# Ryan-Yanlong/DREAM-GNN

Hardware: AMD Instinct MI355X
Metric: GCMC+FGCN SpMM edges/sec and achieved HBM GB/s at 1/2/4/8 MI355X (higher is better)
Workload: dtype f32

## Files before the change

dream_gnn_amd/csrc/dgmi_api.hip:

```cpp
#include <hip/hip_runtime.h>
#include <limits.h>
#include <stdlib.h>
#include <string.h>

#include "dgmi.h"
#include "dgmi_bf16.h"
#include "dgmi_keep.h"
#include "dgmi_layout.h"
#include "dgmi_scale.h"
#include "dgmi_kernels.h"
#include "dgmi_tuning.h"

namespace {

inline hipStream_t as_stream(dgmi_stream_t s) { return static_cast<hipStream_t>(s); }

inline int from_hip(hipError_t e) { return e == hipSuccess ? DGMI_OK : DGMI_ERR_LAUNCH; }

long long env_ll(const char* name, long long dflt) {
  const char* e = getenv(name);
  return e != nullptr && e[0] != '\0' ? atoll(e) : dflt;
}

}

namespace dgmi {

Tuning& tuning() {
  static Tuning t = [] {
    Tuning v;
    v.sliced_rows = (int)env_ll("DGMI_SLICED_ROWS", 0);
    v.sliced_touch_lead = (int)env_ll("DGMI_SLICED_PF", -1);
    v.sliced_lpr = (int)env_ll("DGMI_SLICED_LPR", 0);
    v.sliced_no_off32 = getenv("DGMI_NO_OFF32") != nullptr ? 1 : 0;
    v.sliced_chunk_rows = env_ll("DGMI_SLICED_CHUNK_ROWS", 0);
    v.sliced_taper_rows = env_ll("DGMI_SLICED_TAPER_ROWS", 0);
    v.sliced_owned = (int)env_ll("DGMI_SLICED_OWNED", -1);
    v.sliced_owned_grid = (int)env_ll("DGMI_SLICED_OWNED_GRID", 0);
    v.sliced_owned_wgs = (int)env_ll("DGMI_SLICED_OWNED_WGS", 0);
    v.sliced_owned_rows = (int)env_ll("DGMI_SLICED_OWNED_ROWS", 0);
    v.sliced_owned_lds_rows = env_ll("DGMI_SLICED_OWNED_LDS_ROWS", 0);
    v.sliced_owned_workers = (int)env_ll("DGMI_SLICED_OWNED_WORKERS", 0);
    v.sliced_owned_slices = (int)env_ll("DGMI_SLICED_OWNED_SLICES", 0);
    v.sliced_owned_scaled = (int)env_ll("DGMI_SLICED_OWNED_SCALED", -1);
    v.sliced_owned_lag = (int)env_ll("DGMI_SLICED_OWNED_LAG", -2);
    v.sliced_owned_spin_ticks = env_ll("DGMI_SLICED_OWNED_SPIN_TICKS", 0);
    v.select_window_min = env_ll("DGMI_SELECT_WINDOW_MIN", 0);
    v.select_narrow_window = env_ll("DGMI_SELECT_NARROW_WINDOW", 0) != 0 ? 1 : 0;
    v.sort_plain_tiles = env_ll("DGMI_SORT_PLAIN_TILES", 0) != 0 ? 1 : 0;
    v.knn_screen_first = env_ll("DGMI_KNN_SCREEN_V1", 0) != 0 ? 1 : 0;
    v.knn_pool_chunks = env_ll("DGMI_KNN_POOL_CHUNKS", 0);
    return v;
  }();
  return t;
}

}

extern "C" {

DGMI_API int dgmi_set_tuning(const char* name, int64_t value) {
  if (name == nullptr) return DGMI_ERR_INVALID_ARG;
  dgmi::Tuning& t = dgmi::tuning();
  if (strcmp(name, "sliced_rows") == 0) t.sliced_rows = (int)value;
  else if (strcmp(name, "sliced_touch_lead") == 0) t.sliced_touch_lead = (int)value;
  else if (strcmp(name, "sliced_lpr") == 0) t.sliced_lpr = (int)value;
  else if (strcmp(name, "sliced_no_off32") == 0) t.sliced_no_off32 = value != 0;
  else if (strcmp(name, "sliced_chunk_rows") == 0) t.sliced_chunk_rows = value;
  else if (strcmp(name, "sliced_taper_rows") == 0) t.sliced_taper_rows = value;
  else if (strcmp(name, "sliced_owned") == 0) t.sliced_owned = (int)value;
  else if (strcmp(name, "sliced_owned_grid") == 0) t.sliced_owned_grid = (int)value;
  else if (strcmp(name, "sliced_owned_wgs") == 0) t.sliced_owned_wgs = (int)value;
  else if (strcmp(name, "sliced_owned_rows") == 0) t.sliced_owned_rows = (int)value;
  else if (strcmp(name, "sliced_owned_lds_rows") == 0) t.sliced_owned_lds_rows = value;
  else if (strcmp(name, "sliced_owned_workers") == 0) t.sliced_owned_workers = (int)value;
  else if (strcmp(name, "sliced_owned_slices") == 0) t.sliced_owned_slices = (int)value;
  else if (strcmp(name, "sliced_owned_scaled") == 0) t.sliced_owned_scaled = (int)value;
  else if (strcmp(name, "sliced_owned_lag") == 0) t.sliced_owned_lag = (int)value;
  else if (strcmp(name, "sliced_owned_spin_ticks") == 0) t.sliced_owned_spin_ticks = value;
  else if (strcmp(name, "select_window_min") == 0) t.select_window_min = value;
  else if (strcmp(name, "select_narrow_window") == 0) t.select_narrow_window = value != 0;
  else if (strcmp(name, "sort_plain_tiles") == 0) t.sort_plain_tiles = value != 0;
  else if (strcmp(name, "knn_screen_first") == 0) t.knn_screen_first = value != 0;
  else if (strcmp(name, "knn_pool_chunks") == 0) t.knn_pool_chunks = value;
  else return DGMI_ERR_INVALID_ARG;
  return DGMI_OK;
}

DGMI_API int dgmi_abi_version(void) { return DGMI_ABI_VERSION; }

DGMI_API const char* dgmi_status_string(int status) {
  switch (status) {
    case DGMI_OK: return "ok";
    case DGMI_ERR_INVALID_ARG: return "invalid argument (null pointer, negative size or ld < F)";
    case DGMI_ERR_TOO_LARGE: return "size does not fit the int32 id space";
    case DGMI_ERR_WORKSPACE: return "workspace missing or too small";
    case DGMI_ERR_LAUNCH: return "HIP launch failed";
    case DGMI_ERR_NO_DEVICE: return "no gfx950 device visible";
    default: return "unknown dgmi status";
  }
}

DGMI_API int dgmi_device_ok(void) {
  int n = 0;
  if (hipGetDeviceCount(&n) != hipSuccess || n <= 0) return 0;
  int dev = 0;
  if (hipGetDevice(&dev) != hipSuccess) return 0;
  hipDeviceProp_t prop;
  if (hipGetDeviceProperties(&prop, dev) != hipSuccess) return 0;
  return strncmp(prop.gcnArchName, "gfx950", 6) == 0 ? 1 : 0;
}

DGMI_API int dgmi_csr_from_coo_i32(const int32_t* row, const int32_t* col, int64_t E, int64_t n_rows,
                          int64_t n_cols, int32_t* indptr, int32_t* indices, int32_t* eid, void* workspace,
                          size_t* workspace_bytes, dgmi_stream_t stream) {
  if (E < 0 || n_rows < 0 || workspace_bytes == nullptr) return DGMI_ERR_INVALID_ARG;
  if (E > INT32_MAX || n_rows >= INT32_MAX || n_cols >= INT32_MAX) return DGMI_ERR_TOO_LARGE;
  if (workspace != nullptr) {
    if (indptr == nullptr) return DGMI_ERR_INVALID_ARG;
    if (E > 0 && (row == nullptr || col == nullptr || indices == nullptr || eid == nullptr))
      return DGMI_ERR_INVALID_ARG;
  }
  size_t need = 0;
  hipError_t err = dgmi::csr_from_coo_i32(row, col, E, n_rows, n_cols, indptr, indices, eid, nullptr,
                                          &need, as_stream(stream));
  if (err != hipSuccess) return DGMI_ERR_LAUNCH;
  if (workspace == nullptr) {
    *workspace_bytes = need;
    return DGMI_OK;
  }
// ... 487 lines not shown
```

dream_gnn_amd/csrc/dgmi_owned.hip:

```cpp
#include <hip/hip_runtime.h>
#include <limits.h>
#include <stdint.h>

#include <map>
#include <mutex>
#include <type_traits>
#include <utility>

#include "dgmi_owned_common.h"
#include "dgmi_owned_kernel.h"
#include "dgmi_sliced_common.h"

namespace dgmi {
namespace {

constexpr int64_t kOwnedSpinTicks = 3000;
constexpr int64_t kOwnedMinRows = 32768;
constexpr int kOwnedLag = -1;
constexpr int kOwnedWideSlices = 16;
constexpr int kOwnedAssumedCus = 256;

template <int LPR, int VALS, bool OFF32, int WAVES>
__global__ __launch_bounds__(kWave* WAVES, WAVES == kOwnedWaves ? 4 : 6) void spmm_owned_kernel(
    const int32_t* __restrict__ segptr, const int32_t* __restrict__ indices, const float* __restrict__ X, int64_t ldx,
    const float* __restrict__ dst_scale, float* __restrict__ Y, int64_t ldy, int64_t n_dst, int F, OwnedPlan pl,
    unsigned* __restrict__ arrive, int lag, int64_t spin_ticks, int workers, Epilogue ep) {
  owned_body<OwnedRowF32, LPR, VALS, OFF32, WAVES, true>(segptr, indices, X, ldx, dst_scale, Y, ldy, n_dst, F, pl, arrive, lag,
                                                         spin_ticks, workers, ep);
}

template <int LPR, int VALS, bool OFF32>
__global__ __launch_bounds__(kWave* kOwnedWaves, 4) void spmm_owned_bf16_kernel(
    const int32_t* __restrict__ segptr, const int32_t* __restrict__ indices, const uint16_t* __restrict__ X, int64_t ldx,
    const float* __restrict__ dst_scale, float* __restrict__ Y, int64_t ldy, int64_t n_dst, int F, OwnedPlan pl,
    unsigned* __restrict__ arrive, int lag, int64_t spin_ticks, int workers, Epilogue ep) {
  owned_body<OwnedRowBf16, LPR, VALS, OFF32, kOwnedWaves, false>(segptr, indices, X, ldx, dst_scale, Y, ldy, n_dst, F, pl, arrive,
                                                                 lag, spin_ticks, workers, ep);
}

constexpr size_t kOwnedScaleLdsBytes = sizeof(float) << kScaleBits;
template <int LPR, int VALS>
__global__ __launch_bounds__(kWave* kOwnedWaves, 4) void spmm_owned_scaled_kernel(
    const int32_t* __restrict__ segptr, const int32_t* __restrict__ indices, const float* __restrict__ X, int64_t ldx,
    const float* __restrict__ dst_scale, float* __restrict__ Y, int64_t ldy, int64_t n_dst, int F, OwnedPlan pl, int workers,
    Epilogue ep, const float* __restrict__ table, int n_codes) {
  owned_body<OwnedRowF32, LPR, VALS, true, kOwnedWaves, false, true>(segptr, indices, X, ldx, dst_scale, Y, ldy, n_dst, F, pl, nullptr,
                                                                     -1, 0, workers, ep, table, n_codes);
}

constexpr bool owned_scaled_built(int lpr) { return lpr == 16 || lpr == 32; }

template <int LPR>
hipError_t launch_owned_scaled(const SlicedArgs& a, const OwnedPlan& pl, int64_t grid, hipStream_t s) {
  const int workers = tuning().sliced_owned_workers > 0 && tuning().sliced_owned_workers < kOwnedWorkers ? tuning().sliced_owned_workers : 0;
  const size_t lds = pl.lds_bytes + kOwnedScaleLdsBytes;
#define DGMI_OWNED_SCALED(V)                                                                                              \
  do {                                                                                                                    \
    auto kern = &spmm_owned_scaled_kernel<LPR, V>;                                                                        \
    static const hipError_t attr =                                                                                        \
        hipFuncSetAttribute(reinterpret_cast<const void*>(kern), hipFuncAttributeMaxDynamicSharedMemorySize, 160 << 10);  \
    if (attr != hipSuccess) return attr;                                                                                  \
    hipLaunchKernelGGL(kern, dim3((unsigned)grid), dim3(kWave* kOwnedWaves), lds, s, a.segptr, a.indices,                 \
                       static_cast<const float*>(a.X), a.ldx, a.dst_scale, a.Y, a.ldy, a.n_dst, (int)a.F, pl, workers, a.ep, \
                       a.scale_table, a.n_codes);                                                                         \
  } while (0)
  if (a.id_mult) DGMI_OWNED_SCALED(2); else DGMI_OWNED_SCALED(0);
#undef DGMI_OWNED_SCALED
  return hipGetLastError();
}

template <typename Row, int LPR, int VALS, bool OFF32, int WAVES>
constexpr auto owned_kernel() {
  if constexpr (std::is_same<Row, OwnedRowBf16>::value)
    return &spmm_owned_bf16_kernel<LPR, VALS, OFF32>;
  else
    return &spmm_owned_kernel<LPR, VALS, OFF32, WAVES>;
}

int device_cus() {
  static const int cus = [] {
    int dev = 0, n = 0;
    if (hipGetDevice(&dev) != hipSuccess || hipDeviceGetAttribute(&n, hipDeviceAttributeMultiprocessorCount, dev) != hipSuccess)
      return 0;
    return n;
  }();
  return cus;
}

int owned_class_form(const OwnedPlan& pl, bool id_mult, int64_t table_bytes, int x_bytes) {
  const auto mib = [&](int64_t lo, int64_t hi) { return table_bytes >= (lo << 20) && table_bytes <= (hi << 20); };
  if (x_bytes == 2) {
    if (pl.slices != kOwnedSlices || pl.col_rounds != 1) return 0;
    if (pl.row_rounds == 1 && !id_mult && mib(16, 32)) return 1;
    if (pl.row_rounds == 2 && !id_mult && mib(8, 16)) return 1;
    if (pl.row_rounds == 2 && id_mult && mib(16, 32)) return 1;
    if (pl.row_rounds == 1 && id_mult && mib(8, 16)) return 1;
    return 0;
  }
  if (x_bytes != 4) return 0;
  if (pl.slices == kOwnedSlices) {
    if (pl.col_rounds == 1 && pl.row_rounds == 2 && !id_mult && mib(16, 32)) return 1;
    if (pl.col_rounds == 2 && pl.row_rounds == 1 && id_mult && mib(48, 64)) return 1;
    if (pl.col_rounds == 1 && pl.row_rounds == 1 && id_mult && mib(16, 32)) return 1;
  }
  if (pl.slices == kOwnedWideSlices && pl.col_rounds == 1 && pl.row_rounds == 1 && !id_mult && mib(48, 64)) return 1;
  return 0;
}

int owned_class_phase_tasks(const OwnedPlan& pl, bool id_mult, int64_t table_bytes, int x_bytes) {
  if (x_bytes != 4) return kOwnedPhaseTasks;
  const auto mib = [&](int64_t lo, int64_t hi) { return table_bytes >= (lo << 20) && table_bytes <= (hi << 20); };
  if (pl.slices != kOwnedSlices) return kOwnedPhaseTasks;
  if (pl.col_rounds == 2 && pl.row_rounds == 1 && id_mult && mib(48, 64)) return kOwnedPhaseTasksMult;
  if (pl.col_rounds == 1 && pl.row_rounds == 1 && id_mult && mib(16, 32)) return kOwnedPhaseTasksMult;
  return kOwnedPhaseTasks;
}

bool owned_coresident(const void* kern, int threads, size_t lds, int wgs) {
  static std::mutex mu;
  static std::map<std::pair<const void*, size_t>, int> known;
  std::lock_guard<std::mutex> lock(mu);
// ... 25 lines not shown
    auto kern = owned_kernel<Row, LPR, V, O, WAVES>();                                                                    \
    static const hipError_t attr = hipFuncSetAttribute(reinterpret_cast<const void*>(kern),                               \
                                                       hipFuncAttributeMaxDynamicSharedMemorySize, (160 << 10) / kWgsPerCu); \
    if (attr != hipSuccess) return attr;                                                                                  \
    if (kWgsPerCu > 1 && !owned_coresident(reinterpret_cast<const void*>(kern), kWave * WAVES, pl.lds_bytes, kWgsPerCu)) { \
      *resident = false;                                                                                                  \
      return hipSuccess;                                                                                                  \
    }                                                                                                                     \
    if (lag >= 0) {                                                            \
      const hipError_t err = hipMemsetAsync(arrive, 0, sizeof(unsigned) * 8 * (size_t)pl.phases, s);                      \
      if (err != hipSuccess) return err;                                                                                  \
    }                                                                                                                     \
    hipLaunchKernelGGL(kern, dim3((unsigned)grid), dim3(kWave* WAVES), pl.lds_bytes, s, a.segptr, a.indices,              \
                       static_cast<const typename Row::Elem*>(a.X), a.ldx, a.dst_scale, a.Y, a.ldy, a.n_dst, (int)a.F, pl, \
                       arrive, lag, spin_ticks, workers, a.ep);                                                           \
    }                                                                                                                     \
  } while (0)
  if (a.id_mult) {
    if (off32) DGMI_OWNED(2, true); else DGMI_OWNED(2, false);
  } else {
    if (off32) DGMI_OWNED(0, true); else DGMI_OWNED(0, false);
  }
#undef DGMI_OWNED
  return hipGetLastError();
}

template <typename Row, int WAVES>
hipError_t launch_owned_width(const SlicedArgs& a, const OwnedPlan& pl, int lpr, int64_t grid, bool off32, int lag,
                              int64_t spin_ticks, hipStream_t s, bool* resident) {
  switch (lpr) {
    case 8: return launch_owned<Row, 8, WAVES>(a, pl, grid, off32, lag, spin_ticks, s, resident);
    case 16: return launch_owned<Row, 16, WAVES>(a, pl, grid, off32, lag, spin_ticks, s, resident);
    case 32: return launch_owned<Row, 32, WAVES>(a, pl, grid, off32, lag, spin_ticks, s, resident);
    case 64:
      if constexpr (Row::kMaxLpr >= 64)
        return launch_owned<Row, 64, WAVES>(a, pl, grid, off32, lag, spin_ticks, s, resident);
      else
        return hipErrorInvalidValue;
    default: return hipErrorInvalidValue;
  }
}

bool owned_class_scaled(const OwnedPlan& pl, bool id_mult, int64_t table_bytes) {
  const auto mib = [&](int64_t lo, int64_t hi) { return table_bytes >= (lo << 20) && table_bytes <= (hi << 20); };
  if (pl.slices == kOwnedSlices) {
    if (pl.col_rounds == 1 && pl.row_rounds == 2 && !id_mult && mib(16, 32)) return true;
    if (pl.col_rounds == 2 && pl.row_rounds == 1 && id_mult && mib(48, 64)) return true;
    if (pl.col_rounds == 1 && pl.row_rounds == 1 && id_mult && mib(16, 32)) return true;
  }
  if (pl.slices == kOwnedWideSlices && pl.col_rounds == 1 && pl.row_rounds == 1 && !id_mult && mib(48, 64)) return true;
  return false;
}

hipError_t owned_try(const SlicedArgs& a, hipStream_t s, bool* taken, bool launch);

}

hipError_t spmm_owned_try(const SlicedArgs& a, hipStream_t s, bool* taken) {
  *taken = false;
  if (a.scale_table != nullptr) return hipErrorInvalidValue;
  return owned_try(a, s, taken, true);
}

bool spmm_owned_scaled_takes(const SlicedArgs& a) {
  bool taken = false;
  return a.scale_table != nullptr && owned_try(a, nullptr, &taken, false) == hipSuccess && taken;
}

hipError_t spmm_owned_scaled(const SlicedArgs& a, hipStream_t s, bool* taken) {
  *taken = false;
  if (a.scale_table == nullptr) return hipErrorInvalidValue;
  return owned_try(a, s, taken, true);
}

namespace {

hipError_t owned_try(const SlicedArgs& a, hipStream_t s, bool* taken, bool launch) {
  *taken = false;
  const Tuning& tune = tuning();
  if (tune.sliced_owned == 0) return hipSuccess;
  if ((a.x_bytes != 4 && a.x_bytes != 2) || a.vals != nullptr || a.src_scale != nullptr || a.n_keep != 0 || a.n_slices < 1 || a.n_slices > kOwnedMaxSlices ||
      tune.sliced_chunk_rows > 0 || a.chunk_rows < a.n_dst || a.n_dst == 0 || a.F == 0)
    return hipSuccess;
  if (a.x_bytes == 2 && tune.sliced_owned_slices > 0) return hipSuccess;
  const int64_t grid = tune.sliced_owned_grid > 0 ? tune.sliced_owned_grid : device_cus();
  if (grid < 1) return hipSuccess;
  const int lpr = sliced_lpr(a.F, a.n_src, a.n_slices, a.n_dst, a.full_width, a.n_keep, a.x_bytes, tune.sliced_lpr);
  const int slices = (int)a.n_slices;
  const int cols = 16 / a.x_bytes;
  const int64_t table_bytes = a.n_src * a.ldx * (int64_t)a.x_bytes;
  OwnedPlan pl = owned_plan(a.n_dst, a.F, lpr, grid, tune.sliced_owned_rows, tune.sliced_owned_lds_rows, 1, kOwnedPhaseTasks, slices, cols);
  const int phase_tasks = a.n_dst < kOwnedMinRows ? kOwnedPhaseTasks : owned_class_phase_tasks(pl, a.id_mult, table_bytes, a.x_bytes);
  if (pl.ok && phase_tasks != kOwnedPhaseTasks)
    pl = owned_plan(a.n_dst, a.F, lpr, grid, tune.sliced_owned_rows, tune.sliced_owned_lds_rows, 1, phase_tasks, slices, cols);
  if (!pl.ok || pl.lds_bytes > (size_t)(160 << 10)) return hipSuccess;
  const int rule = a.n_dst < kOwnedMinRows ? 0 : owned_class_form(pl, a.id_mult, table_bytes, a.x_bytes);
  if (tune.sliced_owned != 1 && rule == 0) return hipSuccess;
  const bool off32 = !tune.sliced_no_off32 && (a.n_src * a.ldx + a.F) * a.x_bytes < ((int64_t)1 << 32);
  bool resident = true;
  if (a.scale_table != nullptr) {
    const bool wanted = tune.sliced_owned_scaled == 1 ||
                        (tune.sliced_owned_scaled < 0 && (tune.sliced_owned == 1 || (rule == 1 && owned_class_scaled(pl, a.id_mult, table_bytes))));
    if (!wanted || a.x_bytes != 4 || a.n_src > ((int64_t)1 << kScaleShift) || a.n_codes < 1 || a.n_codes > (1 << kScaleBits) ||
        !off32 || !owned_scaled_built(lpr) || pl.lds_bytes + kOwnedScaleLdsBytes > (size_t)(160 << 10) || tune.sliced_owned_lag >= 0 ||
        tune.sliced_owned_wgs == 2)
      return hipSuccess;
    *taken = true;
    if (!launch) return hipSuccess;
    return lpr == 16 ? launch_owned_scaled<16>(a, pl, grid, s) : launch_owned_scaled<32>(a, pl, grid, s);
  }
  if (!launch) return hipSuccess;
  if (a.x_bytes == 2) {
    *taken = true;
    return launch_owned_width<OwnedRowBf16, kOwnedWaves>(a, pl, lpr, grid, off32, -1, 0, s, &resident);
  }
  const auto arrive_fits = [&](const OwnedPlan& p) {
    return sizeof(unsigned) * 8 * (size_t)p.phases <= sizeof(float) * (size_t)a.n_slices * (size_t)a.n_dst * (size_t)a.ldp;
  };
  if (!arrive_fits(pl)) return hipSuccess;
  const int form = tune.sliced_owned_wgs == 1 || tune.sliced_owned_wgs == 2 ? tune.sliced_owned_wgs : (rule == 2 ? 2 : 1);
  const int64_t spin = tune.sliced_owned_spin_ticks > 0 ? tune.sliced_owned_spin_ticks : kOwnedSpinTicks;
  const int lag = tune.sliced_owned_lag >= -1 ? tune.sliced_owned_lag : kOwnedLag;
  *taken = true;
  if (form == 2) {
    const int64_t grid2 = tune.sliced_owned_grid > 0 ? grid : 2 * grid;
    const OwnedPlan pl2 = owned_plan(a.n_dst, a.F, lpr, grid2, tune.sliced_owned_rows, tune.sliced_owned_lds_rows, 2, kOwnedPhaseTasks, slices);
    if (pl2.ok && pl2.lds_bytes <= (size_t)(80 << 10) && arrive_fits(pl2)) {
      const hipError_t err = launch_owned_width<OwnedRowF32, kOwnedPairWaves>(a, pl2, lpr, grid2, off32, lag, spin, s, &resident);
      if (err != hipSuccess || resident) return err;
    }
  }
  return launch_owned_width<OwnedRowF32, kOwnedWaves>(a, pl, lpr, grid, off32, lag, spin, s, &resident);
}

}

int sliced_layout_slices(int64_t n_dst, int64_t n_src, int64_t F, bool id_mult) {
  const Tuning& tune = tuning();
  if (n_dst < 1 || n_src < 1 || F < 1 || F % 4 != 0 || tune.sliced_owned == 0 || tune.sliced_chunk_rows > 0) return kOwnedSlices;
  const int forced = tune.sliced_owned_slices;
  const int slices = forced > 0 ? (forced < kOwnedMaxSlices ? forced : kOwnedMaxSlices) : kOwnedWideSlices;
  if (slices == kOwnedSlices) return kOwnedSlices;
  if (n_dst * slices >= INT32_MAX || n_dst * slices * F * (int64_t)sizeof(float) > ((int64_t)4096 << 20)) return kOwnedSlices;
  const int64_t grid = tune.sliced_owned_grid > 0 ? tune.sliced_owned_grid : (device_cus() > 0 ? device_cus() : kOwnedAssumedCus);
  const int lpr = sliced_lpr(F, n_src, slices, n_dst, false, 0, 4, tune.sliced_lpr);
  const OwnedPlan pl = owned_plan(n_dst, F, lpr, grid, tune.sliced_owned_rows, tune.sliced_owned_lds_rows, 1, kOwnedPhaseTasks, slices);
  if (!pl.ok || pl.lds_bytes > (size_t)(160 << 10)) return kOwnedSlices;
  if (forced > 0) return slices;
  if (n_dst < kOwnedMinRows) return kOwnedSlices;
  return owned_class_form(pl, id_mult, n_src * F * (int64_t)sizeof(float), 4) == 1 ? slices : kOwnedSlices;
}

}
```

dream_gnn_amd/csrc/dgmi_owned_common.h:

```cpp
#pragma once
#include <hip/hip_runtime.h>
#include <stddef.h>
#include <stdint.h>

namespace dgmi {

constexpr int kOwnedSlices = 8;
constexpr int kOwnedMaxSlices = 64;
constexpr int kOwnedWaves = 16;
constexpr int kOwnedWorkers = kOwnedWaves - 1;
constexpr int kOwnedPairWaves = 12;
constexpr int64_t kOwnedLdsRowBytes = 144 << 10;
constexpr int kOwnedMaxPhases = 128;
constexpr int kOwnedPhaseTasks = 24;
constexpr int kOwnedPhaseTasksMult = 32;
constexpr int kOwnedMaxRows = 8;

struct OwnedPlan {
  bool ok;
  int lpr, G, R;
  int col_rounds, row_rounds, phases;
  int slices;
  int64_t wg_rows;
  int64_t active;
  int round_rows;
  int tasks;
  int64_t n_dst;
  size_t lds_bytes;
};

struct OwnedPhase {
  int col_round, row_round, slice;
};

struct OwnedTask {
  int64_t row0;
  int lds_row;
  int rows;
};

__host__ __device__ constexpr int owned_form_waves(int wgs_per_cu) { return wgs_per_cu == 2 ? kOwnedPairWaves : kOwnedWaves; }

__host__ __device__ inline OwnedPlan owned_plan(int64_t n_dst, int64_t F, int lpr, int64_t grid, int R_req, int64_t lds_rows_cap,
                                                int wgs_per_cu = 1, int phase_tasks_target = kOwnedPhaseTasks,
                                                int slices = kOwnedSlices, int cols_per_lane = 4) {
  OwnedPlan p{};
  p.ok = false;
  p.n_dst = n_dst;
  if (n_dst < 1 || F < 1 || grid < 1 || (wgs_per_cu != 1 && wgs_per_cu != 2) || (lpr != 8 && lpr != 16 && lpr != 32 && lpr != 64) ||
      slices < 1 || slices > kOwnedMaxSlices || (cols_per_lane != 4 && cols_per_lane != 8))
    return p;
  p.lpr = lpr;
  p.slices = slices;
  p.G = 64 / lpr;
  p.col_rounds = (int)((F + cols_per_lane * lpr - 1) / (cols_per_lane * lpr));
  p.wg_rows = (n_dst + grid - 1) / grid;
  p.active = (n_dst + p.wg_rows - 1) / p.wg_rows;
  int64_t fit = kOwnedLdsRowBytes / wgs_per_cu / (4 * cols_per_lane * lpr);
  if (lds_rows_cap > 0 && lds_rows_cap < fit) fit = lds_rows_cap;
  const int64_t rounds = (p.wg_rows + fit - 1) / fit;
  if (rounds * p.col_rounds * slices > kOwnedMaxPhases) return p;
  p.row_rounds = (int)rounds;
  p.round_rows = (int)((p.wg_rows + rounds - 1) / rounds);
  p.phases = p.col_rounds * p.row_rounds * slices;
  int R = R_req;
  if (R <= 0) {
    const int phase_tasks = (phase_tasks_target * (owned_form_waves(wgs_per_cu) - 1) + kOwnedWorkers / 2) / kOwnedWorkers;
    R = (p.round_rows + phase_tasks * p.G / 2) / (phase_tasks * p.G);
    if (R > kOwnedMaxRows) R = kOwnedMaxRows;
  }
  if (R > lpr - 1) R = lpr - 1;
  if (R < 1) R = 1;
  p.R = R;
  p.tasks = (p.round_rows + p.G * R - 1) / (p.G * R);
  p.lds_bytes = (size_t)p.round_rows * 4 * cols_per_lane * lpr + sizeof(int) * ((size_t)p.tasks + p.phases + 2);
  p.ok = true;
  return p;
}

__host__ __device__ inline int64_t owned_wg_rows(const OwnedPlan& p, int64_t wg) {
  const int64_t left = p.n_dst - wg * p.wg_rows;
  return left < 0 ? 0 : (left < p.wg_rows ? left : p.wg_rows);
}

__host__ __device__ inline int64_t owned_round_rows(const OwnedPlan& p, int64_t wg, int row_round) {
  const int64_t left = owned_wg_rows(p, wg) - (int64_t)row_round * p.round_rows;
  return left < 0 ? 0 : (left < p.round_rows ? left : p.round_rows);
}

__host__ __device__ inline int owned_wg_tasks(const OwnedPlan& p, int64_t wg) {
  int64_t rows = owned_wg_rows(p, wg);
  if (rows > p.round_rows) rows = p.round_rows;
  return (int)((rows + p.G * p.R - 1) / (p.G * p.R));
}

__host__ __device__ inline OwnedPhase owned_phase(const OwnedPlan& p, int phase) {
  const int cq = phase / p.slices;
  return OwnedPhase{cq / p.row_rounds, cq % p.row_rounds, phase - cq * p.slices};
}

__host__ __device__ inline OwnedTask owned_task(const OwnedPlan& p, int64_t wg, int row_round, int task, int group) {
  const int64_t lds_row = ((int64_t)task * p.G + group) * p.R;
  int64_t rows = owned_round_rows(p, wg, row_round) - lds_row;
  rows = rows < 0 ? 0 : (rows < p.R ? rows : p.R);
  return OwnedTask{wg * p.wg_rows + (int64_t)row_round * p.round_rows + lds_row, (int)lds_row, (int)rows};
}

struct OwnedWork {
  int phase, task, slice, col_round;
  int64_t row_base;
  int lds_row, rows;
};

__host__ __device__ __forceinline__ OwnedWork owned_decode(const OwnedPlan& pl, int64_t wg, int T, int k, int grp) {
  OwnedWork w;
  if (k >= pl.phases * T) {
    w.phase = pl.phases;
    w.task = w.slice = w.col_round = w.lds_row = w.rows = 0;
    w.row_base = 0;
    return w;
  }
  w.phase = k / T;
  w.task = k - w.phase * T;
  const OwnedPhase ph = owned_phase(pl, w.phase);
  w.slice = ph.slice;
  w.col_round = ph.col_round;
  const OwnedTask t = owned_task(pl, wg, ph.row_round, w.task, grp);
  w.row_base = t.row0 - t.lds_row;
  w.lds_row = t.lds_row;
  w.rows = t.rows;
  return w;
}

constexpr int kOwnedWindow = 4;
constexpr int kOwnedWindowFirstBatches = 2;

__host__ __device__ constexpr int owned_window_groups(int L) { return (L + kOwnedWindow - 1) / kOwnedWindow; }

__host__ __device__ constexpr int owned_window_issue_batch(int g) { return g + 1; }
__host__ __device__ constexpr int owned_window_request_batch(int g) { return g + kOwnedWindowFirstBatches; }

__host__ __device__ constexpr int owned_window_id_edge(int batch, int lane, int L) {
  return batch * kOwnedWindow + lane % kOwnedWindow < L ? batch * kOwnedWindow + lane % kOwnedWindow : L - 1;
}

__host__ __device__ constexpr bool owned_carry(int L_a, int L_b) { return L_a > 0 && L_b > 0; }

__host__ __device__ constexpr int owned_carry_slot_edge(int u, int L_b) { return owned_window_id_edge(0, u, L_b); }

__host__ __device__ constexpr int owned_carry_read_group(int L_a) { return owned_window_groups(L_a) >= 3 ? 0 : -1; }

__host__ __device__ constexpr int owned_carry_start_batch() { return owned_window_issue_batch(0); }

}
```

dream_gnn_amd/csrc/dgmi_owned_kernel.h:

```cpp
#pragma once
#include <hip/hip_runtime.h>
#include <stdint.h>

#include <type_traits>

#include "dgmi_owned_common.h"
#include "dgmi_sliced_common.h"

namespace dgmi {
namespace {

constexpr int kOwnedTouchChunk = 4;
constexpr int kOwnedTouchLead = 8;

struct OwnedRowF32 : RowF32 {
  static constexpr int kLaneSlots = 1;
  static constexpr bool kCarry = true;
  static constexpr bool kPeel = true;

  template <int LPR>
  static __device__ __forceinline__ void commit(float4* slot, bool first, const Acc& acc) {
    if (first) {
      *slot = acc;
      return;
    }
    float4 t = *slot;
    t.x += acc.x;
    t.y += acc.y;
    t.z += acc.z;
    t.w += acc.w;
    *slot = t;
  }

  template <int LPR>
  static __device__ __forceinline__ Acc sum(const float4* slot) {
    return *slot;
  }

  static __device__ __forceinline__ void scale(Acc& t, float d) {
    t.x *= d;
    t.y *= d;
    t.z *= d;
    t.w *= d;
  }

  static __device__ __forceinline__ void write(const Acc& t, float* y, const Epilogue& ep, int64_t row, int col) {
    *reinterpret_cast<float4*>(y) = epilogue4(ep, t, row, col);
  }
};

struct OwnedRowBf16 : RowBf16 {
  static constexpr int kLaneSlots = 2;
  static constexpr bool kCarry = false;
  static constexpr bool kPeel = false;

  template <int LPR>
  static __device__ __forceinline__ Acc sum(const float4* slot) {
    return pairs(slot[0], slot[LPR]);
  }

  template <int LPR>
  static __device__ __forceinline__ void commit(float4* slot, bool first, const Acc& acc) {
    Acc t = acc;
    if (!first) {
      const Acc s = sum<LPR>(slot);
#pragma unroll
      for (int k = 0; k < 4; ++k) t.p[k] = s.p[k] + acc.p[k];
    }
    slot[0] = half(t, 0);
    slot[LPR] = half(t, 1);
  }

  static __device__ __forceinline__ void scale(Acc& t, float d) {
#pragma unroll
    for (int k = 0; k < 4; ++k) t.p[k] *= d;
  }

  static __device__ __forceinline__ void write(const Acc& t, float* y, const Epilogue& ep, int64_t row, int col) {
    OwnedRowF32::write(half(t, 0), y, ep, row, col);
    OwnedRowF32::write(half(t, 1), y + 4, ep, row, col + 4);
  }
};

__device__ __forceinline__ float owned_mul_rn(float a, float b) {
  float r;
  asm("v_mul_f32 %0, %1, %2" : "=v"(r) : "v"(a), "v"(b));
  return r;
}

template <typename Row, int LPR, int VALS, bool OFF32, int WAVES, bool GATE, bool SCALED = false>
__device__ __forceinline__ void owned_body(const int32_t* __restrict__ segptr, const int32_t* __restrict__ indices,
                                           const typename Row::Elem* __restrict__ X, int64_t ldx,
                                           const float* __restrict__ dst_scale, float* __restrict__ Y, int64_t ldy,
                                           int64_t n_dst, int F, OwnedPlan pl, unsigned* __restrict__ arrive, int lag,
                                           int64_t spin_ticks, int workers, Epilogue ep,
                                           const float* __restrict__ table = nullptr, int n_codes = 0) {
  typedef typename Row::Elem Elem;
  typedef typename Row::Acc Acc;
  constexpr bool MULT = VALS == 2;
  constexpr int kIdMask = SCALED ? (int)kScaleIdMask : (MULT ? (int)kMultIdMask : 0x7fffffff);
  static_assert(!SCALED || (std::is_same<Elem, float>::value && kScaleShift + kScaleBits <= kMultShift), "an fp32 table; the code lies below the multiplicity");
  constexpr int kRowSlots = Row::kLaneSlots * LPR;
  constexpr bool CARRY = WAVES == kOwnedWaves && MULT && Row::kCarry;
  extern __shared__ float4 lds_rows[];
  const int lane = threadIdx.x & (kWave - 1);
  const int wave = threadIdx.x >> 6;
  const int grp = lane / LPR, glane = lane % LPR, gbase = grp * LPR;
  const int64_t wg = blockIdx.x;
  const int T = owned_wg_tasks(pl, wg);
  if (T == 0) return;
  int* done = reinterpret_cast<int*>(lds_rows + (size_t)pl.round_rows * kRowSlots);
  int* phase_cnt = done + pl.tasks;
  int* counter = phase_cnt + pl.phases;
  int* open = counter + 1;
  for (int i = threadIdx.x; i < pl.tasks + pl.phases + 2; i += blockDim.x) done[i] = 0;
  float* lds_scale = reinterpret_cast<float*>(open + 1);
  if (SCALED)
    for (int i = threadIdx.x; i < (1 << kScaleBits); i += blockDim.x) lds_scale[i] = i < n_codes ? table[i] : 0.f;
  __syncthreads();
  const int total = pl.phases * T;
  const int label = (int)(blockIdx.x & 7u);

  if (wave == WAVES - 1) {
    const unsigned n_label = (unsigned)((pl.active - label + 7) >> 3);
    const unsigned* my_arrive = GATE ? arrive + (size_t)label * pl.phases : nullptr;
    const int chunks_per_phase = (T + kOwnedTouchChunk - 1) / kOwnedTouchChunk, chunks = pl.phases * chunks_per_phase;
    const int last_gate = GATE && lag >= 0 ? pl.phases - 1 : 0;
    int keepalive = 0, touched = 0, opened = 0;
    bool waiting = false;
    uint64_t wait_start = 0;
    while (touched < chunks || opened < last_gate) {
      bool idle = true;
      const int next = __hip_atomic_load(counter, __ATOMIC_RELAXED, __HIP_MEMORY_SCOPE_WORKGROUP);
      if (touched < chunks) {
        const int P = touched / chunks_per_phase, t0 = (touched - P * chunks_per_phase) * kOwnedTouchChunk;
        if (P * T + t0 <= next + kOwnedTouchLead) {
          ++touched;
          idle = false;
          const OwnedPhase ph = owned_phase(pl, P);
          const int64_t in_round = owned_round_rows(pl, wg, ph.row_round);
          const int64_t lds_first = (int64_t)t0 * pl.G * pl.R;
          int64_t lds_last = lds_first + (int64_t)kOwnedTouchChunk * pl.G * pl.R;
          if (lds_last > in_round) lds_last = in_round;
          if (lds_first < lds_last) {
            const int32_t* sp_s = segptr + (int64_t)ph.slice * n_dst;
            const int64_t r_first = owned_task(pl, wg, ph.row_round, t0, 0).row0, r_last = r_first + (lds_last - lds_first);
            const int64_t rp = lane == 0 ? r_first : (lane == 1 ? r_last : r_first + (int64_t)(lane - 1) * 32);
            int v = 0;
            if (rp <= r_last) v = sp_s[rp];
            keepalive ^= v;
            const int e0 = __builtin_amdgcn_readlane(v, 0), e1 = __builtin_amdgcn_readlane(v, 1);
            for (int64_t p = (int64_t)e0 + (int64_t)lane * 32; p < e1; p += (int64_t)kWave * 32) keepalive ^= indices[p];
            asm volatile("" ::"v"(keepalive));
          }
        }
      }
      if (GATE && opened < last_gate) {
        const int P = opened + 1, need = P - 1 - lag;
        bool ok = need < 0 || __hip_atomic_load(&my_arrive[need], __ATOMIC_RELAXED, __HIP_MEMORY_SCOPE_AGENT) >= n_label;
        if (!ok && next >= P * T) {
          const uint64_t now = __builtin_amdgcn_s_memrealtime();
          if (!waiting) {
            waiting = true;
            wait_start = now;
          } else if (now - wait_start >= (uint64_t)spin_ticks) {
            ok = true;
          }
        }
        if (ok) {
          opened = P;
          waiting = false;
          idle = false;
          __hip_atomic_store(open, P, __ATOMIC_RELAXED, __HIP_MEMORY_SCOPE_WORKGROUP);
        }
      }
      if (idle) __builtin_amdgcn_s_sleep(2);
// ... 9 lines not shown
  };
  auto boundaries = [&](const OwnedWork& t) {
    return segptr[t.rows == 0 ? 0 : (int64_t)t.slice * n_dst + t.row_base + (t.lds_row + (glane < t.rows ? glane : t.rows))];
  };
  auto scales = [&](const OwnedWork& t) {
    if (!CARRY || dst_scale == nullptr || t.slice != pl.slices - 1 || t.rows == 0) return 0.f;
    return dst_scale[t.row_base + (t.lds_row + (glane < t.rows ? glane : t.rows - 1))];
  };
  int nxt_idx = 0, nxt_idx1 = 0, rel_b = 0;
  float my_ds = 0.f, nxt_ds = 0.f;
  static_assert(kOwnedWindowFirstBatches == 2, "nxt_idx and nxt_idx1");
  auto hand_over = [&](int b, const OwnedWork& nxt, int& beg, int& end) {
    beg = __shfl(b, gbase, kWave);
    rel_b = b - beg;
    end = beg + __shfl(rel_b, gbase + nxt.rows, kWave);
    if (beg < end) {
      nxt_idx = indices[beg + owned_carry_slot_edge(glane % kOwnedWindow, end - beg)];
      nxt_idx1 = indices[beg + owned_window_id_edge(owned_carry_start_batch(), glane, end - beg)];
    }
    my_ds = nxt_ds;
    nxt_ds = scales(nxt);
  };

  constexpr int W = kOwnedWindow;
  static_assert(W <= 8 && kMultShift == 28 && LPR % W == 0, "at most eight 4-bit multiplicity fields, shifted down from bit 28");
  typename Row::Reg v[W];
  float sc[SCALED ? W : 1];
  int idx[W];
  int nidx[W];
  uint32_t mults = 0, mults_in = 0, nmults = 0;
  bool carried = false;
  auto read_batch = [&](int batch_idx, int (&out)[W], uint32_t& fields) {
#pragma unroll
    for (int u = 0; u < W; ++u) {
      int id = __shfl(batch_idx, gbase + u, kWave);
      if (MULT) {
        fields = (fields >> 4) | ((uint32_t)id & ((uint32_t)kMultMax << kMultShift));
        if (!SCALED) id &= kIdMask;
      }
      out[u] = id;
    }
    if (MULT) asm volatile("" : "+v"(fields));
  };
  auto read_ids = [&](int batch_idx) { read_batch(batch_idx, idx, mults_in); };

  const uint32_t row_bytes = (uint32_t)ldx * (uint32_t)sizeof(Elem);
  auto issue = [&](int u, const Elem* Xcol, int word, uint32_t cbytes) {
    if (SCALED) {
      sc[u] = lds_scale[((uint32_t)word >> kScaleShift) & ((1u << kScaleBits) - 1u)];
      word &= kIdMask;
    }
    v[u] = Row::template load<OFF32>(X, Xcol, word, ldx, row_bytes, cbytes);
  };
  int k = grab();
  OwnedWork w = owned_decode(pl, wg, T, k, grp);
  int e_begin = 0, e_end = 0;
  hand_over(boundaries(w), w, e_begin, e_end);
  int my_rel = rel_b;
  while (k < total) {
    const int L = e_end - e_begin;
    int col = (w.col_round * LPR + glane) * Row::kCols;
    const bool col_ok = col < F;
    if (!col_ok) col = 0;
    const Elem* Xc = X + col;
    const uint32_t col_bytes = (uint32_t)col * (uint32_t)sizeof(Elem);
    if (L > 0 && !carried) {
      read_ids(nxt_idx);
#pragma unroll
      for (int u = 0; u < W; ++u) issue(u, Xc, idx[u], col_bytes);
      mults = mults_in;
    }
    const int k_next = grab();
    const OwnedWork w_next = owned_decode(pl, wg, T, k_next, grp);
    const int next_b = boundaries(w_next);
    int n_begin = 0, n_end = 0;
    if (GATE && lag >= 0)
      while (__hip_atomic_load(open, __ATOMIC_RELAXED, __HIP_MEMORY_SCOPE_WORKGROUP) < w.phase) __builtin_amdgcn_s_sleep(1);
    while (__hip_atomic_load(&done[w.task], __ATOMIC_ACQUIRE, __HIP_MEMORY_SCOPE_WORKGROUP) < w.phase) __builtin_amdgcn_s_sleep(1);
    const int first_ids = nxt_idx1;
    static_assert(owned_carry_start_batch() == 1, "nxt_idx1");
    if (CARRY) hand_over(next_b, w_next, n_begin, n_end);

    const int nr = w.rows;
    float4* slot = lds_rows + (size_t)w.lds_row * kRowSlots + glane;
    auto commit = [&](int r, const Acc& acc) { Row::template commit<LPR>(slot + r * kRowSlots, w.slice == 0, acc); };
    auto write_rows = [&]() {
      if (w.slice != pl.slices - 1) return;
      for (int r = 0; r < nr; ++r) {
        float d = 0.f;
        if (CARRY) d = __shfl(my_ds, gbase + r, kWave);
        if (!col_ok) continue;
        Acc t = Row::template sum<LPR>(slot + r * kRowSlots);
        const int64_t row = w.row_base + (w.lds_row + r);
        if (dst_scale != nullptr) {
          if (!CARRY) d = dst_scale[row];
          Row::scale(t, d);
        }
        Row::write(t, Y + row * ldy + col, ep, row, col);
      }
    };

    bool carry = false;
    int r = 0;
    Acc acc = Row::zero();
    if (L > 0) {
      int row_end = e_begin + __shfl(my_rel, gbase + 1, kWave);
      auto add = [&](int u) {
        float m = 1.f;
        if (MULT) {
          m = (float)(((mults >> (32 - 4 * W)) & (uint32_t)kMultMax) + 1u);
          mults >>= 4;
        }
        if constexpr (SCALED) {
          const float s = sc[u];
          const float4 t = make_float4(owned_mul_rn(s, v[u].x), owned_mul_rn(s, v[u].y), owned_mul_rn(s, v[u].z), owned_mul_rn(s, v[u].w));
          Row::template add<MULT>(acc, m, t);
        } else {
          Row::template add<MULT>(acc, m, v[u]);
        }
      };
      auto rows_before = [&](int p) {
        while (p >= row_end) {
          commit(r, acc);
          acc = Row::zero();
          ++r;
// ... 100 lines not shown
```

dream_gnn_amd/csrc/dgmi_tuning.h:

```cpp
#pragma once
#include <stdint.h>

namespace dgmi {

struct Tuning {
  int sliced_rows = 0;
  int sliced_touch_lead = -1;
  int sliced_lpr = 0;
  int sliced_no_off32 = 0;
  int64_t sliced_chunk_rows = 0;
  int64_t sliced_taper_rows = 0;
  int sliced_owned = -1;
  int sliced_owned_grid = 0;
  int sliced_owned_wgs = 0;
  int sliced_owned_rows = 0;
  int64_t sliced_owned_lds_rows = 0;
  int sliced_owned_workers = 0;
  int sliced_owned_slices = 0;
  int sliced_owned_scaled = -1;
  int sliced_owned_lag = -2;
  int64_t sliced_owned_spin_ticks = 0;
  int64_t select_window_min = 0;
  int select_narrow_window = 0;
  int sort_plain_tiles = 0;
  int knn_screen_first = 0;
  int64_t knn_pool_chunks = 0;
};

Tuning& tuning();

}
```

Measured before the change: 37.92 billion.

## Replace dedicated toucher wave with duty-rotated prefetch touches in owned SpMM

Adds a duty variant of the owned SpMM kernel where all 16 waves are workers. Instead of one wave dedicated to prefetch-touching segptr and indices, whichever worker grabs a task at a chunk boundary touches the next chunk's boundaries and ids. The goal is to reclaim the idle toucher wave's compute slot and raise worker count, at the cost of adding prefetch latency to some workers' critical path. It is enabled by default only for specific plan shapes and table sizes when no lag gate is used.

```diff
diff --git a/dream_gnn_amd/csrc/dgmi_api.hip b/dream_gnn_amd/csrc/dgmi_api.hip
--- a/dream_gnn_amd/csrc/dgmi_api.hip
+++ b/dream_gnn_amd/csrc/dgmi_api.hip
@@ -43,6 +43,9 @@
     v.sliced_owned_workers = (int)env_ll("DGMI_SLICED_OWNED_WORKERS", 0);
     v.sliced_owned_slices = (int)env_ll("DGMI_SLICED_OWNED_SLICES", 0);
     v.sliced_owned_scaled = (int)env_ll("DGMI_SLICED_OWNED_SCALED", -1);
+    v.sliced_owned_duty = (int)env_ll("DGMI_SLICED_OWNED_DUTY", -1);
+    v.sliced_owned_duty_chunk = (int)env_ll("DGMI_SLICED_OWNED_DUTY_CHUNK", 0);
+    v.sliced_owned_duty_lead = (int)env_ll("DGMI_SLICED_OWNED_DUTY_LEAD", 0);
     v.sliced_owned_lag = (int)env_ll("DGMI_SLICED_OWNED_LAG", -2);
     v.sliced_owned_spin_ticks = env_ll("DGMI_SLICED_OWNED_SPIN_TICKS", 0);
     v.select_window_min = env_ll("DGMI_SELECT_WINDOW_MIN", 0);
@@ -76,6 +79,9 @@
   else if (strcmp(name, "sliced_owned_workers") == 0) t.sliced_owned_workers = (int)value;
   else if (strcmp(name, "sliced_owned_slices") == 0) t.sliced_owned_slices = (int)value;
   else if (strcmp(name, "sliced_owned_scaled") == 0) t.sliced_owned_scaled = (int)value;
+  else if (strcmp(name, "sliced_owned_duty") == 0) t.sliced_owned_duty = (int)value;
+  else if (strcmp(name, "sliced_owned_duty_chunk") == 0) t.sliced_owned_duty_chunk = (int)value;
+  else if (strcmp(name, "sliced_owned_duty_lead") == 0) t.sliced_owned_duty_lead = (int)value;
   else if (strcmp(name, "sliced_owned_lag") == 0) t.sliced_owned_lag = (int)value;
   else if (strcmp(name, "sliced_owned_spin_ticks") == 0) t.sliced_owned_spin_ticks = value;
   else if (strcmp(name, "select_window_min") == 0) t.select_window_min = value;
diff --git a/dream_gnn_amd/csrc/dgmi_owned.hip b/dream_gnn_amd/csrc/dgmi_owned.hip
--- a/dream_gnn_amd/csrc/dgmi_owned.hip
+++ b/dream_gnn_amd/csrc/dgmi_owned.hip
@@ -48,25 +48,56 @@
                                                                      -1, 0, workers, ep, table, n_codes);
 }
 
+template <int LPR, int VALS, bool SCALED>
+__global__ __launch_bounds__(kWave* kOwnedWaves, 4) void spmm_owned_duty_kernel(
+    const int32_t* __restrict__ segptr, const int32_t* __restrict__ indices, const float* __restrict__ X, int64_t ldx,
+    const float* __restrict__ dst_scale, float* __restrict__ Y, int64_t ldy, int64_t n_dst, int F, OwnedPlan pl, int workers,
+    Epilogue ep, const float* __restrict__ table, int n_codes, int duty_chunk, int duty_lead) {
+  owned_body<OwnedRowF32, LPR, VALS, true, kOwnedWaves, false, SCALED, true>(segptr, indices, X, ldx, dst_scale, Y, ldy, n_dst, F, pl,
+                                                                             nullptr, -1, 0, workers, ep, table, n_codes, duty_chunk,
+                                                                             duty_lead);
+}
+
 constexpr bool owned_scaled_built(int lpr) { return lpr == 16 || lpr == 32; }
+constexpr bool owned_duty_built(int lpr) { return owned_scaled_built(lpr); }
+
+int owned_tuned_workers(int all) {
+  const int w = tuning().sliced_owned_workers;
+  return w > 0 && w < all ? w : 0;
+}
+
+template <auto KERN, typename... Extra>
+hipError_t launch_owned_tabled(const SlicedArgs& a, const OwnedPlan& pl, int64_t grid, size_t lds, int workers, hipStream_t s,
+                               Extra... extra) {
+  static const hipError_t attr =
+      hipFuncSetAttribute(reinterpret_cast<const void*>(KERN), hipFuncAttributeMaxDynamicSharedMemorySize, 160 << 10);
+  if (attr != hipSuccess) return attr;
+  hipLaunchKernelGGL(KERN, dim3((unsigned)grid), dim3(kWave* kOwnedWaves), lds, s, a.segptr, a.indices,
+                     static_cast<const float*>(a.X), a.ldx, a.dst_scale, a.Y, a.ldy, a.n_dst, (int)a.F, pl, workers, a.ep,
+                     a.scale_table, a.n_codes, extra...);
+  return hipGetLastError();
+}
 
 template <int LPR>
 hipError_t launch_owned_scaled(const SlicedArgs& a, const OwnedPlan& pl, int64_t grid, hipStream_t s) {
-  const int workers = tuning().sliced_owned_workers > 0 && tuning().sliced_owned_workers < kOwnedWorkers ? tuning().sliced_owned_workers : 0;
   const size_t lds = pl.lds_bytes + kOwnedScaleLdsBytes;
-#define DGMI_OWNED_SCALED(V)                                                                                              \
-  do {                                                                                                                    \
-    auto kern = &spmm_owned_scaled_kernel<LPR, V>;                                                                        \
-    static const hipError_t attr =                                                                                        \
-        hipFuncSetAttribute(reinterpret_cast<const void*>(kern), hipFuncAttributeMaxDynamicSharedMemorySize, 160 << 10);  \
-    if (attr != hipSuccess) return attr;                                                                                  \
-    hipLaunchKernelGGL(kern, dim3((unsigned)grid), dim3(kWave* kOwnedWaves), lds, s, a.segptr, a.indices,                 \
-                       static_cast<const float*>(a.X), a.ldx, a.dst_scale, a.Y, a.ldy, a.n_dst, (int)a.F, pl, workers, a.ep, \
-                       a.scale_table, a.n_codes);                                                                         \
-  } while (0)
-  if (a.id_mult) DGMI_OWNED_SCALED(2); else DGMI_OWNED_SCALED(0);
-#undef DGMI_OWNED_SCALED
-  return hipGetLastError();
+  const int workers = owned_tuned_workers(kOwnedWorkers);
+  if (a.id_mult) return launch_owned_tabled<&spmm_owned_scaled_kernel<LPR, 2>>(a, pl, grid, lds, workers, s);
+  return launch_owned_tabled<&spmm_owned_scaled_kernel<LPR, 0>>(a, pl, grid, lds, workers, s);
+}
+
+template <int LPR>
+hipError_t launch_owned_duty(const SlicedArgs& a, const OwnedPlan& pl, int64_t grid, hipStream_t s) {
+  const int chunk = tuning().sliced_owned_duty_chunk > 0 ? tuning().sliced_owned_duty_chunk : pl.tasks;
+  const int lead = tuning().sliced_owned_duty_lead > 0 ? tuning().sliced_owned_duty_lead : chunk;
+  const int workers = owned_tuned_workers(kOwnedDutyWorkers);
+  if (a.scale_table != nullptr) {
+    const size_t lds = pl.lds_bytes + kOwnedScaleLdsBytes;
+    if (a.id_mult) return launch_owned_tabled<&spmm_owned_duty_kernel<LPR, 2, true>>(a, pl, grid, lds, workers, s, chunk, lead);
+    return launch_owned_tabled<&spmm_owned_duty_kernel<LPR, 0, true>>(a, pl, grid, lds, workers, s, chunk, lead);
+  }
+  if (a.id_mult) return launch_owned_tabled<&spmm_owned_duty_kernel<LPR, 2, false>>(a, pl, grid, pl.lds_bytes, workers, s, chunk, lead);
+  return launch_owned_tabled<&spmm_owned_duty_kernel<LPR, 0, false>>(a, pl, grid, pl.lds_bytes, workers, s, chunk, lead);
 }
 
 template <typename Row, int LPR, int VALS, bool OFF32, int WAVES>
@@ -198,6 +229,17 @@
   return false;
 }
 
+bool owned_class_duty(const OwnedPlan& pl, bool id_mult, int64_t table_bytes) {
+  const auto mib = [&](int64_t lo, int64_t hi) { return table_bytes >= (lo << 20) && table_bytes <= (hi << 20); };
+  if (pl.slices == kOwnedSlices) {
+    if (pl.col_rounds == 1 && pl.row_rounds == 2 && !id_mult && mib(16, 32)) return true;
+    if (pl.col_rounds == 2 && pl.row_rounds == 1 && id_mult && mib(48, 64)) return true;
+    if (pl.col_rounds == 1 && pl.row_rounds == 1 && id_mult && mib(16, 32)) return true;
+  }
+  if (pl.slices == kOwnedWideSlices && pl.col_rounds == 1 && pl.row_rounds == 1 && !id_mult && mib(48, 64)) return true;
+  return false;
+}
+
 hipError_t owned_try(const SlicedArgs& a, hipStream_t s, bool* taken, bool launch);
 
 }
@@ -244,6 +286,13 @@
   if (tune.sliced_owned != 1 && rule == 0) return hipSuccess;
   const bool off32 = !tune.sliced_no_off32 && (a.n_src * a.ldx + a.F) * a.x_bytes < ((int64_t)1 << 32);
   bool resident = true;
+  const int lag = tune.sliced_owned_lag >= -1 ? tune.sliced_owned_lag : kOwnedLag;
+  OwnedPlan pl_duty{};
+  if (a.x_bytes == 4 && off32 && owned_duty_built(lpr) && lag < 0 && tune.sliced_owned_wgs != 2 && rule != 2 &&
+      (tune.sliced_owned_duty == 1 || (tune.sliced_owned_duty < 0 && rule == 1 && owned_class_duty(pl, a.id_mult, table_bytes)))) {
+    pl_duty = owned_plan(a.n_dst, a.F, lpr, grid, tune.sliced_owned_rows, tune.sliced_owned_lds_rows, 1, phase_tasks, slices, cols, kOwnedDutyWorkers);
+    if (pl_duty.lds_bytes + (a.scale_table != nullptr ? kOwnedScaleLdsBytes : 0) > (size_t)(160 << 10)) pl_duty.ok = false;
+  }
   if (a.scale_table != nullptr) {
     const bool wanted = tune.sliced_owned_scaled == 1 ||
                         (tune.sliced_owned_scaled < 0 && (tune.sliced_owned == 1 || (rule == 1 && owned_class_scaled(pl, a.id_mult, table_bytes))));
@@ -253,12 +302,17 @@
       return hipSuccess;
     *taken = true;
     if (!launch) return hipSuccess;
+    if (pl_duty.ok) return lpr == 16 ? launch_owned_duty<16>(a, pl_duty, grid, s) : launch_owned_duty<32>(a, pl_duty, grid, s);
     return lpr == 16 ? launch_owned_scaled<16>(a, pl, grid, s) : launch_owned_scaled<32>(a, pl, grid, s);
   }
   if (!launch) return hipSuccess;
   if (a.x_bytes == 2) {
     *taken = true;
     return launch_owned_width<OwnedRowBf16, kOwnedWaves>(a, pl, lpr, grid, off32, -1, 0, s, &resident);
+  }
+  if (pl_duty.ok) {
+    *taken = true;
+    return lpr == 16 ? launch_owned_duty<16>(a, pl_duty, grid, s) : launch_owned_duty<32>(a, pl_duty, grid, s);
   }
   const auto arrive_fits = [&](const OwnedPlan& p) {
     return sizeof(unsigned) * 8 * (size_t)p.phases <= sizeof(float) * (size_t)a.n_slices * (size_t)a.n_dst * (size_t)a.ldp;
@@ -266,7 +320,6 @@
   if (!arrive_fits(pl)) return hipSuccess;
   const int form = tune.sliced_owned_wgs == 1 || tune.sliced_owned_wgs == 2 ? tune.sliced_owned_wgs : (rule == 2 ? 2 : 1);
   const int64_t spin = tune.sliced_owned_spin_ticks > 0 ? tune.sliced_owned_spin_ticks : kOwnedSpinTicks;
-  const int lag = tune.sliced_owned_lag >= -1 ? tune.sliced_owned_lag : kOwnedLag;
   *taken = true;
   if (form == 2) {
     const int64_t grid2 = tune.sliced_owned_grid > 0 ? grid : 2 * grid;
diff --git a/dream_gnn_amd/csrc/dgmi_owned_common.h b/dream_gnn_amd/csrc/dgmi_owned_common.h
--- a/dream_gnn_amd/csrc/dgmi_owned_common.h
+++ b/dream_gnn_amd/csrc/dgmi_owned_common.h
@@ -9,6 +9,7 @@
 constexpr int kOwnedMaxSlices = 64;
 constexpr int kOwnedWaves = 16;
 constexpr int kOwnedWorkers = kOwnedWaves - 1;
+constexpr int kOwnedDutyWorkers = kOwnedWaves;
 constexpr int kOwnedPairWaves = 12;
 constexpr int64_t kOwnedLdsRowBytes = 144 << 10;
 constexpr int kOwnedMaxPhases = 128;
@@ -43,12 +44,14 @@
 
 __host__ __device__ inline OwnedPlan owned_plan(int64_t n_dst, int64_t F, int lpr, int64_t grid, int R_req, int64_t lds_rows_cap,
                                                 int wgs_per_cu = 1, int phase_tasks_target = kOwnedPhaseTasks,
-                                                int slices = kOwnedSlices, int cols_per_lane = 4) {
+                                                int slices = kOwnedSlices, int cols_per_lane = 4, int workers = 0) {
   OwnedPlan p{};
   p.ok = false;
   p.n_dst = n_dst;
+  if (workers == 0) workers = owned_form_waves(wgs_per_cu) - 1;
   if (n_dst < 1 || F < 1 || grid < 1 || (wgs_per_cu != 1 && wgs_per_cu != 2) || (lpr != 8 && lpr != 16 && lpr != 32 && lpr != 64) ||
-      slices < 1 || slices > kOwnedMaxSlices || (cols_per_lane != 4 && cols_per_lane != 8))
+      slices < 1 || slices > kOwnedMaxSlices || (cols_per_lane != 4 && cols_per_lane != 8) || workers < 1 ||
+      workers > owned_form_waves(wgs_per_cu))
     return p;
   p.lpr = lpr;
   p.slices = slices;
@@ -65,7 +68,7 @@
   p.phases = p.col_rounds * p.row_rounds * slices;
   int R = R_req;
   if (R <= 0) {
-    const int phase_tasks = (phase_tasks_target * (owned_form_waves(wgs_per_cu) - 1) + kOwnedWorkers / 2) / kOwnedWorkers;
+    const int phase_tasks = (phase_tasks_target * workers + kOwnedWorkers / 2) / kOwnedWorkers;
     R = (p.round_rows + phase_tasks * p.G / 2) / (phase_tasks * p.G);
     if (R > kOwnedMaxRows) R = kOwnedMaxRows;
   }
@@ -152,4 +155,59 @@
 
 __host__ __device__ constexpr int owned_carry_start_batch() { return owned_window_issue_batch(0); }
 
-}
+constexpr int kOwnedTouchChunk = 4;
+constexpr int kOwnedTouchLead = 8;
+constexpr int kOwnedTouchLineWords = 32;
+
+__host__ __device__ constexpr int owned_touch_chunks(int T, int chunk) { return (T + chunk - 1) / chunk; }
+
+struct OwnedTouchRows {
+  bool any;
+  int slice;
+  int64_t r_first, r_last;
+};
+
+__host__ __device__ inline OwnedTouchRows owned_touch_rows(const OwnedPlan& pl, int64_t wg, int T, int chunk, int c) {
+  const int per_phase = owned_touch_chunks(T, chunk);
+  const int P = c / per_phase, t0 = (c - P * per_phase) * chunk;
+  const OwnedPhase ph = owned_phase(pl, P);
+  const int64_t in_round = owned_round_rows(pl, wg, ph.row_round);
+  const int64_t lds_first = (int64_t)t0 * pl.G * pl.R;
+  int64_t lds_last = lds_first + (int64_t)chunk * pl.G * pl.R;
+  if (lds_last > in_round) lds_last = in_round;
+  OwnedTouchRows r{lds_first < lds_last, ph.slice, 0, 0};
+  if (r.any) {
+    r.r_first = owned_task(pl, wg, ph.row_round, t0, 0).row0;
+    r.r_last = r.r_first + (lds_last - lds_first);
+  }
+  return r;
+}
+
+__host__ __device__ constexpr int64_t owned_touch_boundary(int64_t r_first, int64_t r_last, int64_t j) {
+  return j == 0 ? r_first : (j == 1 ? r_last : (r_first + (j - 1) * kOwnedTouchLineWords <= r_last ? r_first + (j - 1) * kOwnedTouchLineWords : -1));
+}
+
+__host__ __device__ constexpr int64_t owned_touch_id(int64_t e0, int64_t e1, int64_t j) {
+  return e0 + j * kOwnedTouchLineWords < e1 ? e0 + j * kOwnedTouchLineWords : -1;
+}
+
+__host__ __device__ inline int owned_duty_chunk(int k, int T, int chunk, int phases) {
+  if (k < 0 || T < 1 || k >= phases * T) return -1;
+  const int P = k / T, t = k - P * T;
+  return t % chunk == 0 ? P * owned_touch_chunks(T, chunk) + t / chunk : -1;
+}
+
+__host__ __device__ constexpr int owned_duty_lead_chunks(int lead, int chunk) { return (lead + chunk - 1) / chunk; }
+
+struct OwnedDutySpan {
+  int first, end;
+};
+
+__host__ __device__ inline OwnedDutySpan owned_duty_span(int c, int chunks, int lead_chunks) {
+  OwnedDutySpan s{c == 0 ? 0 : c + lead_chunks, c + lead_chunks + 1};
+  if (s.end > chunks) s.end = chunks;
+  if (s.first > s.end) s.first = s.end;
+  return s;
+}
+
+}
diff --git a/dream_gnn_amd/csrc/dgmi_owned_kernel.h b/dream_gnn_amd/csrc/dgmi_owned_kernel.h
--- a/dream_gnn_amd/csrc/dgmi_owned_kernel.h
+++ b/dream_gnn_amd/csrc/dgmi_owned_kernel.h
@@ -9,9 +9,6 @@
 
 namespace dgmi {
 namespace {
-
-constexpr int kOwnedTouchChunk = 4;
-constexpr int kOwnedTouchLead = 8;
 
 struct OwnedRowF32 : RowF32 {
   static constexpr int kLaneSlots = 1;
@@ -88,13 +85,15 @@
   return r;
 }
 
-template <typename Row, int LPR, int VALS, bool OFF32, int WAVES, bool GATE, bool SCALED = false>
+template <typename Row, int LPR, int VALS, bool OFF32, int WAVES, bool GATE, bool SCALED = false, bool DUTY = false>
 __device__ __forceinline__ void owned_body(const int32_t* __restrict__ segptr, const int32_t* __restrict__ indices,
                                            const typename Row::Elem* __restrict__ X, int64_t ldx,
                                            const float* __restrict__ dst_scale, float* __restrict__ Y, int64_t ldy,
                                            int64_t n_dst, int F, OwnedPlan pl, unsigned* __restrict__ arrive, int lag,
                                            int64_t spin_ticks, int workers, Epilogue ep,
-                                           const float* __restrict__ table = nullptr, int n_codes = 0) {
+                                           const float* __restrict__ table = nullptr, int n_codes = 0, int duty_chunk = 0,
+                                           int duty_lead = 0) {
+  static_assert(!DUTY || !GATE, "the phase gate lives in the toucher");
   typedef typename Row::Elem Elem;
   typedef typename Row::Acc Acc;
   constexpr bool MULT = VALS == 2;
@@ -121,7 +120,7 @@
   const int total = pl.phases * T;
   const int label = (int)(blockIdx.x & 7u);
 
-  if (wave == WAVES - 1) {
+  if (!DUTY && wave == WAVES - 1) {
     const unsigned n_label = (unsigned)((pl.active - label + 7) >> 3);
     const unsigned* my_arrive = GATE ? arrive + (size_t)label * pl.phases : nullptr;
     const int chunks_per_phase = (T + kOwnedTouchChunk - 1) / kOwnedTouchChunk, chunks = pl.phases * chunks_per_phase;
@@ -237,7 +236,36 @@
     }
     v[u] = Row::template load<OFF32>(X, Xcol, word, ldx, row_bytes, cbytes);
   };
+  const int duty_chunks = DUTY ? pl.phases * owned_touch_chunks(T, duty_chunk) : 0;
+  const int duty_lead_chunks = DUTY ? owned_duty_lead_chunks(duty_lead, duty_chunk) : 0;
+  auto duty = [&](int slot) {
+    const int c = owned_duty_chunk(slot, T, duty_chunk, pl.phases);
+    if (c < 0) return;
+    const OwnedDutySpan span = owned_duty_span(c, duty_chunks, duty_lead_chunks);
+    int keepalive = 0;
+    for (int cc = span.first; cc < span.end; ++cc) {
+      const OwnedTouchRows tr = owned_touch_rows(pl, wg, T, duty_chunk, cc);
+      if (!tr.any) continue;
+      const int32_t* sp_s = segptr + (int64_t)tr.slice * n_dst;
+      int v = 0;
+      for (int64_t j = lane;; j += kWave) {
+        const int64_t rp = owned_touch_boundary(tr.r_first, tr.r_last, j);
+        if (rp < 0) break;
+        const int b = sp_s[rp];
+        if (j < 2) v = b;
+        keepalive ^= b;
+      }
+      const int e0 = __builtin_amdgcn_readlane(v, 0), e1 = __builtin_amdgcn_readlane(v, 1);
+      for (int64_t j = lane;; j += kWave) {
+        const int64_t p = owned_touch_id(e0, e1, j);
+        if (p < 0) break;
+        keepalive ^= indices[p];
+      }
+    }
+    asm volatile("" ::"v"(keepalive));
+  };
   int k = grab();
+  if (DUTY) duty(k);
   OwnedWork w = owned_decode(pl, wg, T, k, grp);
   int e_begin = 0, e_end = 0;
   hand_over(boundaries(w), w, e_begin, e_end);
@@ -256,6 +284,7 @@
       mults = mults_in;
     }
     const int k_next = grab();
+    if (DUTY) duty(k_next);
     const OwnedWork w_next = owned_decode(pl, wg, T, k_next, grp);
     const int next_b = boundaries(w_next);
     int n_begin = 0, n_end = 0;
diff --git a/dream_gnn_amd/csrc/dgmi_tuning.h b/dream_gnn_amd/csrc/dgmi_tuning.h
--- a/dream_gnn_amd/csrc/dgmi_tuning.h
+++ b/dream_gnn_amd/csrc/dgmi_tuning.h
@@ -18,6 +18,9 @@
   int sliced_owned_workers = 0;
   int sliced_owned_slices = 0;
   int sliced_owned_scaled = -1;
+  int sliced_owned_duty = -1;
+  int sliced_owned_duty_chunk = 0;
+  int sliced_owned_duty_lead = 0;
   int sliced_owned_lag = -2;
   int64_t sliced_owned_spin_ticks = 0;
   int64_t select_window_min = 0;
```

After: 38.69 billion (median of 6 runs). 1.02x the previous value.
